# jaredhuling/oem

Measured on NVIDIA B200. Metric: full lambda-path fit time, lower is better.
Workload: dtype f64

## Files before the change

oem_b200/build.py:

```python
import os
import subprocess
import sys

HERE = os.path.dirname(os.path.abspath(__file__))
CSRC = os.path.join(HERE, "csrc")
LIBDIR = os.path.join(HERE, "lib")
LIB = os.path.join(LIBDIR, "liboem_b200.so")
SOURCES = ["runtime.cu", "gram_syrk.cu", "colstats.cu", "assemble.cu", "path_kernel.cu", "host_common.cu",
           "entries.cu", "entry_logistic.cu", "entry_xval.cu", "entry_xval_logistic.cu", "entry_sparse.cu", "cvscore.cu", "logit_slab.cu", "comm.cu", "ingest.cu"]
NVCC_FLAGS = ["-gencode", "arch=compute_100a,code=sm_100a", "-lineinfo", "-O3", "-std=c++17",
              "-Xcompiler", "-fPIC", "-Xcompiler", "-O2"]


def _stale(target, deps):
    if not os.path.exists(target):
        return True
    t = os.path.getmtime(target)
    return any(os.path.getmtime(d) > t for d in deps)


def build(force=False, verbose=False):
    nvcc = os.environ.get("NVCC", "/usr/local/cuda/bin/nvcc")
    os.makedirs(LIBDIR, exist_ok=True)
    objdir = os.path.join(HERE, "build")
    os.makedirs(objdir, exist_ok=True)
    headers = [os.path.join(CSRC, f) for f in os.listdir(CSRC) if f.endswith((".h", ".cuh"))]
    headers.append(os.path.join(HERE, "..", "include", "oem_b200.h"))
    srcs = [s for s in SOURCES if os.path.exists(os.path.join(CSRC, s))]
    objs, procs = [], []
    for s in srcs:
        src = os.path.join(CSRC, s)
        obj = os.path.join(objdir, s.replace(".cu", ".o"))
        objs.append(obj)
        if force or _stale(obj, [src] + headers):
            cmd = [nvcc] + NVCC_FLAGS + (["-Xptxas", "-v"] if verbose else []) + ["-c", src, "-o", obj]
            procs.append((s, subprocess.Popen(cmd, stdout=subprocess.PIPE, stderr=subprocess.STDOUT, text=True)))
    failed = False
    for s, pr in procs:
        out, _ = pr.communicate()
        if pr.returncode != 0 or verbose:
            sys.stderr.write(f"--- nvcc {s} ---\n{out}\n")
        failed = failed or pr.returncode != 0
    if failed:
        raise RuntimeError("nvcc failed")
    if procs or force or _stale(LIB, objs):
        cmd = [nvcc, "-shared", "-o", LIB] + objs + ["-gencode", "arch=compute_100a,code=sm_100a"]
        subprocess.check_call(cmd)
    return LIB


if __name__ == "__main__":
    print(build(force="--force" in sys.argv, verbose="-v" in sys.argv))
```

oem_b200/csrc/entries.cu:

```cuda
#include <algorithm>
#include <cmath>
#include <cstdlib>
#include <cstring>
#include "host_common.h"

namespace oemb200 {

thread_local std::string g_last_error;

void check_common(const oemb200_spec *s, const oemb200_opts *o, const oemb200_result *r, const char *want_family,
                  bool allow_weights) {
    if (!s || !o || !r) fail(OEMB200_EINVAL, "spec / opts / result must not be NULL");
    if (!s->family || strcmp(s->family, want_family) != 0) {
        if (strcmp(want_family, "gaussian") == 0)
            fail(OEMB200_EINVAL, "binomial not available for oem_fit_dense, use oem_fit_logistic_dense");
        fail(OEMB200_EINVAL, "family must be \"%s\"", want_family);
    }
    if (s->n_weights > 0 && !allow_weights) fail(OEMB200_EUNSUPPORTED, "weights not implemented yet.");
    if (s->n_weights > 0 && !s->weights) fail(OEMB200_EINVAL, "n_weights > 0 but weights is NULL");
    if (!r->beta || !r->lambda || !r->niter || !r->d) fail(OEMB200_EINVAL, "result buffers beta/lambda/niter/d are required");
    if (o->maxit < 1) fail(OEMB200_EINVAL, "maxit must be >= 1");
}

void to_device_matrix(Ctx &cx, const double *x, int64_t n, int p, int64_t ldx, DevMatrix &m) {
    if (is_device_ptr(x)) { m.p = x; m.ld = ldx; return; }
    size_t free_b = 0, total_b = 0;
    OEM_CUDA(cudaMemGetInfo(&free_b, &total_b));
    m.ld = n + (n & 1);
    const size_t need = (size_t)m.ld * p * 8;
    if (need + (2ull << 30) > free_b)
        fail(OEMB200_EUNSUPPORTED, "x (%.1f GB) does not fit next to the workspace on the device (%.1f GB free); "
             "use oem_fit_big (streams row chunks) or shard the rows over more GPUs", need / 1e9, free_b / 1e9);
    m.own.alloc((size_t)m.ld * p);
    if (m.ld != n) m.own.zero(cx.stream);
    h2d_block(cx, x, ldx, n, p, m.own.p, m.ld, cx.stream);
    m.p = m.own.p;
}
void to_device_vector(Ctx &cx, const double *v, int64_t n, DevVector &d) {
    if (is_device_ptr(v)) { d.p = v; return; }
    d.own.alloc(n + (n & 1));
    d.own.zero(cx.stream);
    d.own.upload(v, n, cx.stream);
    cx.st.h2d_bytes += n * 8;
    d.p = d.own.p;
}

void fill_common_outputs(const Setup &su, oemb200_result *res) {
    const int L = su.Lmax;
    for (int pp = 0; pp < su.P; ++pp) {
        for (int i = 0; i < L; ++i) {
            res->lambda[(size_t)pp * L + i] = i < (int)su.lam[pp].size() ? su.lam[pp][i] : 0.0;
            if (res->loss) res->loss[(size_t)pp * L + i] = 1e99;
        }
        if (res->nlam_out) res->nlam_out[pp] = su.nlam_run[pp];
    }
}

void finish_stats(Ctx &cx, PhaseTimers &tm, size_t total_id, oemb200_result *res) {
    tm.stop(total_id);
    cx.finish();
    if (res->stats) *res->stats = cx.st;
}

static void fit_big(const double *x, int64_t n, int p, int64_t ldx, const double *y, const oemb200_spec *s,
                    const oemb200_opts *o, oemb200_result *res) {
    check_common(s, o, res, "gaussian");
    if (n < 1 || p < 1 || ldx < n) fail(OEMB200_EINVAL, "bad dimensions n=%lld p=%d ldx=%lld", (long long)n, p, (long long)ldx);
    const int icpt = s->intercept ? 1 : 0, q = p + icpt;
    Ctx cx(o);
    PhaseTimers &tm = *cx.tm;
    const size_t t_total = tm.start(&cx.st.ms_total);
    Setup su;
    su.parse(s, q, p, false);

    const size_t nb = (size_t)p * p + 3 * (size_t)p + 3;
    DBuf<double> bundle(nb);
    bundle.zero(cx.stream);
    double *G = bundle.p, *stats = G + (size_t)p * p, *ysum = stats + 3 * (size_t)p, *nobs = ysum + 2;

    DevVector yv;
    to_device_vector(cx, y, n, yv);
    const size_t t_y = tm.start(&cx.st.ms_colstats);
    vecsum_launch(cx, yv.p, n, 0.0, ysum, false);
    tm.stop(t_y);

    const bool fused_stats = getenv("OEMB200_SEPARATE_COLSTATS") == nullptr;
    if (is_device_ptr(x)) {
        if (fused_stats) {
            gram_launch(cx, x, n, p, ldx, {RowSegment{0, n, 0}}, 1, nullptr, nullptr, G, false, yv.p, stats);
        } else {
            const size_t t1 = tm.start(&cx.st.ms_colstats);
            colstats_launch(cx, x, n, p, ldx, nullptr, yv.p, nullptr, stats, false);
            tm.stop(t1);
            gram_launch(cx, x, n, p, ldx, {RowSegment{0, n, 0}}, 1, nullptr, nullptr, G, false);
        }
    } else {
        const double gigs = o->gigs > 0 ? o->gigs : 1.0;
        int64_t rows = (int64_t)(gigs * 1e9 / (8.0 * p));
        const int64_t align = 2 * gram_kt();
        rows = std::max<int64_t>(align, rows / align * align);
        rows = std::min<int64_t>(rows, (n + align - 1) / align * align);
        DBuf<double> stage[2];
        stage[0].alloc((size_t)rows * p);
        stage[1].alloc((size_t)rows * p);
        struct CopyLane {
            cudaStream_t s = nullptr;
            cudaEvent_t ready[2] = {nullptr, nullptr}, freed[2] = {nullptr, nullptr};
            CopyLane() {
                OEM_CUDA(cudaStreamCreateWithFlags(&s, cudaStreamNonBlocking));
                for (int b = 0; b < 2; ++b) {
                    OEM_CUDA(cudaEventCreateWithFlags(&ready[b], cudaEventDisableTiming));
                    OEM_CUDA(cudaEventCreateWithFlags(&freed[b], cudaEventDisableTiming));
                }
            }
            ~CopyLane() {
                if (s) cudaStreamSynchronize(s);
                for (int b = 0; b < 2; ++b) { if (ready[b]) cudaEventDestroy(ready[b]); if (freed[b]) cudaEventDestroy(freed[b]); }
                if (s) cudaStreamDestroy(s);
            }
        } lane;
        cudaStream_t cs = lane.s;
        cudaEvent_t *ready = lane.ready, *freed = lane.freed;
        const int64_t nchunks = (n + rows - 1) / rows;
        const bool pinned_src = is_pinned_host(x);
        auto issue_copy = [&](int64_t c) {
            const int b = (int)(c & 1);
            const int64_t r0 = c * rows, nr = std::min(rows, n - r0);
            if (c >= 2) OEM_CUDA(cudaStreamWaitEvent(cs, freed[b], 0));
            h2d_block(cx, x + r0, ldx, nr, p, stage[b].p, rows, cs);
            OEM_CUDA(cudaEventRecord(ready[b], cs));
        };
        const size_t t_h = tm.start(&cx.st.ms_h2d);
        issue_copy(0);
        if (nchunks > 1 && pinned_src) issue_copy(1);
        for (int64_t c = 0; c < nchunks; ++c) {
            const int b = (int)(c & 1);
            const int64_t r0 = c * rows, nr = std::min(rows, n - r0);
            OEM_CUDA(cudaStreamWaitEvent(cx.stream, ready[b], 0));
            if (fused_stats) {
                gram_launch(cx, stage[b].p, nr, p, rows, {RowSegment{0, nr, 0}}, 1, nullptr, nullptr, G, c > 0, yv.p + r0, stats);
            } else {
                colstats_launch(cx, stage[b].p, nr, p, rows, nullptr, yv.p + r0, nullptr, stats, c > 0);
                gram_launch(cx, stage[b].p, nr, p, rows, {RowSegment{0, nr, 0}}, 1, nullptr, nullptr, G, c > 0);
            }
            OEM_CUDA(cudaEventRecord(freed[b], cx.stream));
            const int64_t nxt = pinned_src ? c + 2 : c + 1;
            if (nxt < nchunks) issue_copy(nxt);
        }
        tm.stop(t_h);
        cx.sync();
    }
    const double nd = (double)n;
    OEM_CUDA(cudaMemcpyAsync(nobs, &nd, 8, cudaMemcpyHostToDevice, cx.stream));
    const size_t t_ar = tm.start(&cx.st.ms_allreduce);
    cx.all_reduce(bundle.p, (int64_t)nb);
    tm.stop(t_ar);

    double n_tot = 0.0;
    OEM_CUDA(cudaMemcpyAsync(&n_tot, nobs, 8, cudaMemcpyDeviceToHost, cx.stream));
    cx.sync();
    if (!(n_tot > q)) fail(OEMB200_EUNSUPPORTED, "n <= p branch (XX' form, src/oem_big.h:363-366) is outside the hot path");

    const size_t t_as = tm.start(&cx.st.ms_assemble);
    DBuf<double> XX((size_t)q * q), XY(q), cinv(p);
    assemble_aug_launch(cx, p, icpt, s->standardize ? 1 : 0, 1, 1, G, stats, ysum, 1, nobs, nobs, XX.p, XY.p, cinv.p, nullptr);
    std::vector<double> hXY(q), hcinv(p);
    XY.download(hXY.data(), q, cx.stream);
    cinv.download(hcinv.data(), p, cx.stream);
    tm.stop(t_as);
    cx.sync();

    double lmax = 0.0;
    for (int j = 0; j < q; ++j) lmax = std::max(lmax, std::fabs(hXY[j]));
    su.build_lambdas(s, lmax, false);

    PenaltyTables tb(cx, su, s, p, icpt);
    PathBuffers pb;
// ... 553 lines not shown
        cudaGetLastError();
        delete m;
    });
}

int oemb200_matrix_info(const oemb200_matrix *m, int64_t *n, int *p, int64_t *ld, const double **dev_ptr, int64_t *h2d_bytes,
                        double *ms_upload) {
    return guarded([&] {
        check_handle(m);
        if (n) *n = m->n;
        if (p) *p = m->p;
        if (ld) *ld = m->ld;
        if (dev_ptr) *dev_ptr = m->dev;
        if (h2d_bytes) *h2d_bytes = m->h2d_bytes;
        if (ms_upload) *ms_upload = m->ms_upload;
    });
}

int oemb200_fit_dense_h(const oemb200_matrix *x, const double *y, const oemb200_spec *spec, const oemb200_opts *opts,
                        oemb200_result *res) {
    return guarded([&] { check_handle(x); HandleOpts h(x, opts); fit_dense(x->dev, x->n, x->p, x->ld, y, spec, &h.o, res); });
}
int oemb200_fit_big_h(const oemb200_matrix *x, const double *y, const oemb200_spec *spec, const oemb200_opts *opts,
                      oemb200_result *res) {
    return guarded([&] { check_handle(x); HandleOpts h(x, opts); fit_big(x->dev, x->n, x->p, x->ld, y, spec, &h.o, res); });
}
int oemb200_fit_logistic_dense_h(const oemb200_matrix *x, const double *y, const oemb200_spec *spec, const oemb200_opts *opts,
                                 oemb200_result *res) {
    return guarded([&] {
        check_handle(x);
        HandleOpts h(x, opts);
        fit_logistic(x->dev, x->n, x->p, x->ld, y, spec, &h.o, res, &x->slab);
    });
}
int oemb200_xval_dense_h(const oemb200_matrix *x, const double *y, const oemb200_spec *spec, int nfolds, const int *foldid,
                         const char *type_measure, const oemb200_opts *opts, oemb200_result *res) {
    return guarded([&] {
        check_handle(x);
        HandleOpts h(x, opts);
        fit_xval(x->dev, x->n, x->p, x->ld, y, spec, nfolds, foldid, type_measure, &h.o, res);
    });
}
int oemb200_xval_logistic_dense_h(const oemb200_matrix *x, const double *y, const oemb200_spec *spec, int nfolds,
                                  const int *foldid, const char *type_measure, const oemb200_opts *opts, oemb200_result *res) {
    return guarded([&] {
        check_handle(x);
        HandleOpts h(x, opts);
        fit_xval_logistic(x->dev, x->n, x->p, x->ld, y, spec, nfolds, foldid, type_measure, &h.o, res);
    });
}
int oemb200_predict_h(const oemb200_matrix *x, const double *beta, int beta_rows, int nlambda, int type, double *out,
                      int64_t ldo, const oemb200_opts *opts, oemb200_stats *stats) {
    return guarded([&] {
        check_handle(x);
        HandleOpts h(x, opts);
        predict_entry(x->dev, x->n, x->p, x->ld, beta, beta_rows, nlambda, type, out, ldo, &h.o, stats);
    });
}

static void phase_ctx_opts(oemb200_opts &o, void *stream) {
    oemb200_default_opts(&o);
    o.stream = stream;
}
static double elapsed_ms(cudaEvent_t a, cudaEvent_t b) {
    float ms = 0.f;
    cudaEventElapsedTime(&ms, a, b);
    return ms;
}
#define OEM_PHASE_TIMED(body)                                                    \
    oemb200_opts o_; phase_ctx_opts(o_, stream);                                 \
    Ctx cx(&o_);                                                                 \
    cudaEvent_t ea, eb;                                                          \
    OEM_CUDA(cudaEventCreate(&ea)); OEM_CUDA(cudaEventCreate(&eb));              \
    OEM_CUDA(cudaEventRecord(ea, cx.stream));                                    \
    body;                                                                        \
    OEM_CUDA(cudaEventRecord(eb, cx.stream));                                    \
    cx.sync();                                                                   \
    if (ms_out) *ms_out = elapsed_ms(ea, eb);                                    \
    cudaEventDestroy(ea); cudaEventDestroy(eb);

int oemb200_gram(const double *x_dev, int64_t n, int p, int64_t ldx, const double *mean_dev, const double *row_w_dev,
                 double *g_dev, void *stream, double *ms_out) {
    return guarded([&] {
        OEM_PHASE_TIMED(gram_launch(cx, x_dev, n, p, ldx, {RowSegment{0, n, 0}}, 1, mean_dev, row_w_dev, g_dev, false));
    });
}
int oemb200_colstats(const double *x_dev, int64_t n, int p, int64_t ldx, const double *v0_dev, const double *v1_dev,
                     double *out_dev, void *stream, double *ms_out) {
    return guarded([&] { OEM_PHASE_TIMED(colstats_launch(cx, x_dev, n, p, ldx, v0_dev, v1_dev, nullptr, out_dev, false)); });
}
int oemb200_xb_logistic(const double *x_dev, int64_t n, int p, int64_t ldx, const double *b_dev, double b0,
                        const double *y_dev, double *prob_dev, double *resid_dev, double *w_dev, void *stream,
                        double *ms_out) {
    return guarded([&] {
        OEM_PHASE_TIMED(xb_launch(cx, x_dev, n, p, ldx, b_dev, b0, y_dev, nullptr, prob_dev, resid_dev, w_dev, true));
    });
}
int oemb200_logit_slab_pass(const double *x_dev, int64_t n, int p, int64_t ldx, const double *b_dev, double b0,
                            const double *y_dev, double *prob_dev, double *w_dev, double *grad_dev, int reps, void *stream,
                            double *ms_out, double *ms_relayout_out) {
    return guarded([&] {
        if (!x_dev || !b_dev || !y_dev || !grad_dev || n < 1 || p < 1 || ldx < n) fail(OEMB200_EINVAL, "logit_slab_pass: bad arguments");
        if (!logit_slab_rows(p)) fail(OEMB200_EUNSUPPORTED, "the slab kernel covers 8 <= p <= 2048 (p = %d)", p);
        oemb200_opts o_; phase_ctx_opts(o_, stream);
        Ctx cx(&o_);
        cudaEvent_t e0, e1, e2;
        OEM_CUDA(cudaEventCreate(&e0)); OEM_CUDA(cudaEventCreate(&e1)); OEM_CUDA(cudaEventCreate(&e2));
        DBuf<double> slabs(logit_slab_doubles(n, p)), d_b0(1);
        OEM_CUDA(cudaMemcpyAsync(d_b0.p, &b0, 8, cudaMemcpyHostToDevice, cx.stream));
        OEM_CUDA(cudaEventRecord(e0, cx.stream));
        logit_slab_relayout(cx, x_dev, n, p, ldx, slabs.p);
        OEM_CUDA(cudaEventRecord(e1, cx.stream));
        const int nrep = reps < 1 ? 1 : reps;
        for (int r = 0; r < nrep; ++r) logit_slab_launch(cx, slabs.p, n, p, b_dev, d_b0.p, y_dev, prob_dev, w_dev, grad_dev);
        OEM_CUDA(cudaEventRecord(e2, cx.stream));
        cx.sync();
        if (ms_relayout_out) *ms_relayout_out = elapsed_ms(e0, e1);
        if (ms_out) *ms_out = elapsed_ms(e1, e2) / nrep;
        cudaEventDestroy(e0); cudaEventDestroy(e1); cudaEventDestroy(e2);
    });
}
int oemb200_logit_fold_pass(const double *x_dev, int64_t n, int p, int64_t ldx, const double *b_dev, const double *b0_dev,
                            const double *y_dev, const int *fold_dev, int M, const int *conv_dev, double *grad_dev, int reps,
                            void *stream, double *ms_out, double *ms_relayout_out, int *sweeps_out) {
    return guarded([&] {
        if (!x_dev || !b_dev || !b0_dev || !y_dev || !fold_dev || !grad_dev || n < 1 || p < 1 || ldx < n || M < 1)
            fail(OEMB200_EINVAL, "logit_fold_pass: bad arguments");
        if (!logit_fold_models(p)) fail(OEMB200_EUNSUPPORTED, "the fused fold pass covers 8 <= p <= 2048 (p = %d)", p);
        oemb200_opts o_; phase_ctx_opts(o_, stream);
        Ctx cx(&o_);
        cudaEvent_t e0, e1, e2;
        OEM_CUDA(cudaEventCreate(&e0)); OEM_CUDA(cudaEventCreate(&e1)); OEM_CUDA(cudaEventCreate(&e2));
        DBuf<double> slabs(logit_fold_doubles(n, p));
        OEM_CUDA(cudaEventRecord(e0, cx.stream));
        logit_fold_relayout(cx, x_dev, n, p, ldx, slabs.p);
        OEM_CUDA(cudaEventRecord(e1, cx.stream));
        const int nrep = reps < 1 ? 1 : reps;
        int sweeps = 0;
        for (int r = 0; r < nrep; ++r)
            sweeps = logit_fold_launch(cx, slabs.p, n, p, b_dev, b0_dev, y_dev, fold_dev, M, conv_dev, nullptr, nullptr, grad_dev);
        OEM_CUDA(cudaEventRecord(e2, cx.stream));
        cx.sync();
        if (ms_relayout_out) *ms_relayout_out = elapsed_ms(e0, e1);
        if (ms_out) *ms_out = elapsed_ms(e1, e2) / nrep;
        if (sweeps_out) *sweeps_out = sweeps;
        cudaEventDestroy(e0); cudaEventDestroy(e1); cudaEventDestroy(e2);
    });
}
int oemb200_top_eig(const double *xx_dev, int q, double *lambda_max_out, int *steps_out, void *stream) {
    return guarded([&] {
        oemb200_opts o_; phase_ctx_opts(o_, stream);
        Ctx cx(&o_);
        DBuf<double> d(1), xy(q);
        DBuf<int> lz(1);
        xy.zero(cx.stream);
        PathProblem pp;
        pp.q = q; pp.ngram = 1; pp.XX = xx_dev; pp.XY = xy.p; pp.d = d.p; pp.compute_eig = true;
        pp.eig_factor = 1.0; pp.eig_tol = 1e-10; pp.Lmax = 1; pp.lanczos_steps = lz.p;
        path_launch(cx, pp);
        double h; int k;
        d.download(&h, 1, cx.stream);
        lz.download(&k, 1, cx.stream);
        cx.sync();
        if (lambda_max_out) *lambda_max_out = h;
        if (steps_out) *steps_out = k;
    });
}
// ... 3 lines not shown
```

oem_b200/csrc/gram_syrk.cu:

```cuda
#include <algorithm>
#include <functional>
#include <cstdlib>
#include <type_traits>
#include <mutex>
#include "runtime.h"

namespace oemb200 {

constexpr int G_TILE = 128;
constexpr int G_KT = 36;
constexpr int G_KSTEPS = G_KT / 4;
constexpr int G_STAGES = 3;
constexpr int G_CWARPS = 8;
constexpr int G_THREADS = G_CWARPS * 32;
constexpr int G_PANEL = G_TILE * G_KT;
constexpr int G_PANEL_BYTES = G_PANEL * 8;
constexpr int G_STAGE_BYTES = 2 * G_PANEL_BYTES;
constexpr int G_SMEM_BYTES = G_STAGES * G_STAGE_BYTES + 128;

int gram_kt() { return G_KT; }

struct GramItem {
    int pi, pj, slot, pad;
    long long row0, row1;
// ... 277 lines not shown
                    so[e * G_TILE + rlo * 8 + g] = st_lo[e];
                    so[e * G_TILE + rhi * 8 + g] = st_hi[e];
                }
            }
        }
        double *slot = ws + (size_t)it.slot * (G_TILE * G_TILE);
#pragma unroll
        for (int sl = 0; sl < 17; ++sl) {
            const int row = sl <= warp ? rlo : rhi;
            const int col = sl <= warp ? sl : sl - warp - 1;
            const int i = row * 8 + g, j = col * 8 + 2 * t;
            slot[(size_t)j * G_TILE + i] = acc[sl][0];
            slot[(size_t)(j + 1) * G_TILE + i] = acc[sl][1];
        }
    }
}

__global__ void __launch_bounds__(256)
gram_reduce_kernel(const double *__restrict__ ws, const GramTile *__restrict__ tiles, double *__restrict__ G, int q,
                   int accumulate) {
    const GramTile tl = tiles[blockIdx.y];
    const int e = blockIdx.x * 256 + threadIdx.x;
    const int i = e & (G_TILE - 1), j = e >> 7;
    const int gi = tl.pi * G_TILE + i, gj = tl.pj * G_TILE + j;
    if (gi >= q || gj >= q || gi < gj) return;
    const double *p = ws + (size_t)tl.slot0 * (G_TILE * G_TILE) + e;
    double s = 0.0;
    for (int k = 0; k < tl.nslots; ++k) s += p[(size_t)k * (G_TILE * G_TILE)];
    double *Go = G + (size_t)tl.out * q * q;
    if (accumulate) s += Go[(size_t)gj * q + gi];
    Go[(size_t)gj * q + gi] = s;
    Go[(size_t)gi * q + gj] = s;
}

__global__ void gram_stats_reduce_kernel(const double *__restrict__ stats_ws, const int *__restrict__ chunk_out, int nchunks,
                                         int npanels, int q, int nout, const double *__restrict__ G,
                                         double *__restrict__ stats_out, int accumulate) {
    const int j = blockIdx.x * blockDim.x + threadIdx.x;
    const int o = blockIdx.y;
    if (j >= q) return;
    const int pi = j / G_TILE, jl = j - pi * G_TILE;
    double s[2] = {0.0, 0.0};
    for (int c = 0; c < nchunks; ++c) {
        if (chunk_out[c] != o) continue;
        const double *so = stats_ws + ((size_t)c * npanels + pi) * (2 * G_TILE) + jl;
#pragma unroll
        for (int e = 0; e < 2; ++e) s[e] += so[e * G_TILE];
    }
    double *out = stats_out + (size_t)o * 3 * q;
#pragma unroll
    for (int e = 0; e < 2; ++e) out[(size_t)e * q + j] = accumulate ? out[(size_t)e * q + j] + s[e] : s[e];
    out[(size_t)2 * q + j] = G[(size_t)o * q * q + (size_t)j * q + j];
}

typedef CUresult (*EncodeTiledFn)(CUtensorMap *, CUtensorMapDataType, cuuint32_t, void *, const cuuint64_t *,
                                  const cuuint64_t *, const cuuint32_t *, const cuuint32_t *, CUtensorMapInterleave,
                                  CUtensorMapSwizzle, CUtensorMapL2promotion, CUtensorMapFloatOOBfill);

static EncodeTiledFn get_encode_fn() {
    static EncodeTiledFn fn = nullptr;
    static std::once_flag once;
    std::call_once(once, [] {
        void *p = nullptr;
        cudaDriverEntryPointQueryResult qres;
        if (cudaGetDriverEntryPoint("cuTensorMapEncodeTiled", &p, cudaEnableDefault, &qres) == cudaSuccess &&
            qres == cudaDriverEntryPointSuccess)
            fn = reinterpret_cast<EncodeTiledFn>(p);
    });
    return fn;
}

template <bool C, bool W, bool T, bool S>
static void launch_variant(Ctx &cx, const CUtensorMap &tm, const double *X, int64_t ld, int64_t n, int q,
                           const GramItem *d_items, int nitems, const double *mean, const double *roww, double *ws,
                           const double *yvec, double *stats_ws, int npanels) {
    auto kern = gram_syrk_kernel<C, W, T, S>;
    OEM_CUDA(cudaFuncSetAttribute(kern, cudaFuncAttributeMaxDynamicSharedMemorySize, G_SMEM_BYTES));
    kern<<<nitems, G_THREADS, G_SMEM_BYTES, cx.stream>>>(tm, X, ld, n, q, d_items, mean, roww, ws, yvec, stats_ws, npanels);
    OEM_CUDA(cudaGetLastError());
}

void gram_launch(Ctx &cx, const double *X, int64_t n, int q, int64_t ld, const std::vector<RowSegment> &segs,
                 int nout, const double *mean, const double *roww, double *G, bool accumulate, const double *stats_y,
                 double *stats_out) {
    if (stats_out && roww) fail(OEMB200_EINVAL, "gram: fused column statistics are not available with row weights");
    if (n <= 0 || q <= 0) fail(OEMB200_EINVAL, "gram: empty matrix (n=%lld, p=%d)", (long long)n, q);
    if (n >= (1ll << 31)) fail(OEMB200_EINVAL, "gram: more than 2^31-1 rows per call; shard or chunk the rows");
    const int P = (q + G_TILE - 1) / G_TILE;
    const int ntile_pairs = P * (P + 1) / 2;

    int64_t rows_total = 0;
    for (auto &s : segs) {
        if (s.row0 < 0 || s.row1 > n || s.row1 < s.row0 || s.out < 0 || s.out >= nout)
            fail(OEMB200_EINVAL, "gram: bad row segment");
        if ((s.row0 % G_KT) != 0 && s.row0 != 0) fail(OEMB200_EINVAL, "gram: segment start not a multiple of %d", G_KT);
        if (((s.row1 - s.row0) % G_KT) != 0 && s.row1 != n)
            fail(OEMB200_EINVAL, "gram: interior segment length not a multiple of %d", G_KT);
        rows_total += s.row1 - s.row0;
    }
    const int64_t min_rows = 32 * G_KT;
    auto round_chunk = [&](int64_t target_chunks) {
        int64_t cr = (rows_total + target_chunks - 1) / std::max<int64_t>(1, target_chunks);
        return std::max<int64_t>(min_rows, ((cr + G_KT - 1) / G_KT) * G_KT);
    };
    int64_t chunk_rows;
    if (const char *e = getenv("OEMB200_GRAM_WAVES")) {
        chunk_rows = round_chunk(std::max<int64_t>(1, (int64_t)std::max(1, atoi(e)) * cx.num_sms / ntile_pairs));
    } else {
        const bool partial = (q % G_TILE) != 0;
        const int nfull = partial ? (P - 1) * (P - 2) / 2 : P * (P - 1) / 2;
        const int nlast = partial ? P - 1 : 0;
        const double cost_last = partial ? (8.0 + std::max(0, std::min(8, (q - (P - 1) * G_TILE - 64 + 7) / 8)) +
                                            std::min(8, (q - (P - 1) * G_TILE + 7) / 8) - 8.0) / 16.0 : 1.0;
        const double cost_diag = stats_out ? 0.60 : 0.54;
        auto makespan = [&](int64_t cr) {
            std::vector<double> cost;
            std::vector<double> len;
            for (auto &sg : segs) {
                const int64_t l = sg.row1 - sg.row0;
                if (l <= 0) continue;
                const int64_t nc = (l + cr - 1) / cr;
                const int64_t per = (((l + nc - 1) / nc) + G_KT - 1) / G_KT * G_KT;
                for (int64_t r = 0; r < l; r += per) len.push_back((double)((std::min(l, r + per) - r + G_KT - 1) / G_KT) + 3.0);
            }
            for (double c : {1.0, cost_last, cost_diag}) {
                const int nt = c == 1.0 ? nfull : (c == cost_diag ? P : nlast);
                for (double l : len)
                    for (int t = 0; t < nt; ++t) cost.push_back(l * c);
            }
            std::vector<double> sm(cx.num_sms, 0.0);
            std::make_heap(sm.begin(), sm.end(), std::greater<double>());
            double end = 0.0;
            for (double c : cost) {
                std::pop_heap(sm.begin(), sm.end(), std::greater<double>());
                sm.back() += c;
                end = std::max(end, sm.back());
                std::push_heap(sm.begin(), sm.end(), std::greater<double>());
            }
            return end;
        };
        const int64_t c_lo = std::max<int64_t>(1, (int64_t)6 * cx.num_sms / ntile_pairs);
        const int64_t c_hi = std::max<int64_t>(c_lo, (int64_t)14 * cx.num_sms / ntile_pairs);
        chunk_rows = round_chunk(c_lo);
        double best = makespan(chunk_rows);
        for (int64_t c = c_lo + 1; c <= c_hi; ++c) {
            const int64_t cr = round_chunk(c);
            if (cr == chunk_rows) continue;
            const double m = makespan(cr);
            if (m < best * 0.999) { best = m; chunk_rows = cr; }
        }
    }
    const int64_t max_slots = (1536ll << 20) / (G_TILE * G_TILE * 8);
    for (;;) {
        int64_t nchunks = 0;
        for (auto &s : segs) nchunks += std::max<int64_t>(1, (s.row1 - s.row0 + chunk_rows - 1) / chunk_rows);
        if (nchunks * ntile_pairs <= max_slots) break;
        chunk_rows *= 2;
    }

    std::vector<GramItem> items;
    std::vector<GramTile> tiles;
    std::vector<int> chunks_per_out(nout, 0);
    struct Chunk { int64_t r0, r1; int out, idx; };
    std::vector<Chunk> chunks;
    for (auto &s : segs) {
        const int64_t len = s.row1 - s.row0;
        if (len == 0) continue;
        const int64_t nc = (len + chunk_rows - 1) / chunk_rows;
        int64_t per = (((len + nc - 1) / nc) + G_KT - 1) / G_KT * G_KT;
        for (int64_t r = s.row0; r < s.row1; r += per) {
// ... 105 lines not shown
```

oem_b200/csrc/runtime.h:

```cpp
#pragma once
#include <cuda_runtime.h>
#include <cstdint>
#include <cstring>
#include <string>
#include <array>
#include <vector>
#include "../../include/oem_b200.h"
#include "common.cuh"

namespace oemb200 {

cudaEvent_t event_acquire();
void event_release(cudaEvent_t e);

struct PhaseTimers {
    struct Rec { cudaEvent_t a, b; double *acc; };
    std::vector<Rec> recs;
    cudaStream_t s;
    bool off = getenv("OEMB200_NO_PHASE_TIMERS") != nullptr;
    explicit PhaseTimers(cudaStream_t s_) : s(s_) {}
    PhaseTimers(const PhaseTimers &) = delete;
    ~PhaseTimers() { for (auto &r : recs) { event_release(r.a); event_release(r.b); } }
    size_t start(double *acc) {
        if (off) return 0;
// ... 28 lines not shown

    explicit Ctx(const oemb200_opts *o);
    ~Ctx();
    void sync() { st.host_syncs += 1; OEM_CUDA(cudaStreamSynchronize(stream)); }
    bool distributed() const { return comm != nullptr || allreduce != nullptr; }
    void all_reduce(double *dev_buf, int64_t count, const int *skip = nullptr, unsigned long long *t_acc = nullptr);
    bool all_reduce_can_skip(int64_t count) const;
    void finish();
};

void *pool_alloc(size_t bytes);
void pool_free(void *p);
void pool_release_all();

template <typename T>
struct DBuf {
    T *p = nullptr;
    size_t n = 0;
    DBuf() {}
    explicit DBuf(size_t n_) { alloc(n_); }
    DBuf(const DBuf &) = delete;
    DBuf &operator=(const DBuf &) = delete;
    DBuf(DBuf &&o) noexcept : p(o.p), n(o.n) { o.p = nullptr; o.n = 0; }
    DBuf &operator=(DBuf &&o) noexcept {
        if (this != &o) { release(); p = o.p; n = o.n; o.p = nullptr; o.n = 0; }
        return *this;
    }
    ~DBuf() { release(); }
    void alloc(size_t n_) {
        release();
        n = n_;
        if (n) p = static_cast<T *>(pool_alloc(n * sizeof(T)));
    }
    void release() {
        if (p) pool_free(p);
        p = nullptr;
        n = 0;
    }
    void zero(cudaStream_t s) { if (n) OEM_CUDA(cudaMemsetAsync(p, 0, n * sizeof(T), s)); }
    void upload(const T *h, size_t cnt, cudaStream_t s) {
        OEM_CUDA(cudaMemcpyAsync(p, h, cnt * sizeof(T), cudaMemcpyHostToDevice, s));
    }
    void download(T *h, size_t cnt, cudaStream_t s) const {
        OEM_CUDA(cudaMemcpyAsync(h, p, cnt * sizeof(T), cudaMemcpyDeviceToHost, s));
    }
};

bool is_device_ptr(const void *p);

template <typename F>
void collective_guard(Ctx &cx, F &&f) {
    int code = 0;
    std::string msg;
    try {
        f();
    } catch (const Error &e) {
        code = e.code;
        msg = e.what();
    }
    if (cx.distributed()) {
        DBuf<double> flag(1);
        double h = code ? 1.0 : 0.0;
        flag.upload(&h, 1, cx.stream);
        cx.sync();
        cx.all_reduce(flag.p, 1);
        flag.download(&h, 1, cx.stream);
        cx.sync();
        if (h > 0.0 && !code) fail(OEMB200_ECOMM, "another rank rejected its inputs; this rank stops before the next collective");
    }
    if (code) throw Error(code, msg);
}

bool is_pinned_host(const void *p);
void h2d_block(Ctx &cx, const double *src, int64_t ldx, int64_t nr, int p, double *dst, int64_t ld_dst, cudaStream_t stream);
void release_host_stager();

void comm_all_reduce(oemb200_comm *c, double *dev_buf, int64_t count, cudaStream_t stream, const int *skip = nullptr,
                     unsigned long long *t_acc = nullptr);
bool comm_can_skip(const oemb200_comm *c, int64_t count);

struct RowSegment { int64_t row0, row1; int out; };
void gram_launch(Ctx &cx, const double *X, int64_t n, int q, int64_t ld, const std::vector<RowSegment> &segs,
                 int nout, const double *mean, const double *roww, double *G, bool accumulate,
                 const double *stats_y = nullptr, double *stats_out = nullptr);
int gram_kt();

void colstats_launch(Ctx &cx, const double *X, int64_t n, int p, int64_t ld, const double *v0, const double *v1,
                     const double *shift, double *out3p, bool accumulate);
void vecsum_launch(Ctx &cx, const double *v, int64_t n, double shift, double *out2, bool accumulate);
void affine_launch(Ctx &cx, const double *v, int64_t n, double shift, double divisor, double *out);
void axpy_launch(Ctx &cx, int64_t n, double a, const double *x, double *y);
void xb_launch(Ctx &cx, const double *X, int64_t n, int p, int64_t ld, const double *b, double b0, const double *y,
               double *eta, double *prob, double *resid, double *w, bool logistic, const double *b0_dev = nullptr);

struct ChainDesc {
    int gram;
    int penalty;
    int nlam;
    int lam_off;
    double alpha, gamma, tau;
    int out_off;
};
struct PathScratch;
PathScratch *path_scratch_create();
void path_scratch_destroy(PathScratch *s);

struct PathProblem {
    int q = 0;
    int ngram = 0;
    const double *XX = nullptr;
    const double *XY = nullptr;
    double *d = nullptr;
    bool compute_eig = true;
    double eig_factor = 1.005;
    double eig_tol = 1e-11;
    std::vector<ChainDesc> chains;
    const double *lambdas = nullptr;
    int Lmax = 0;
    const double *pen_fact = nullptr;
    int ngroups = 0;
    int ngidx = 0;
    const int *unique_groups = nullptr, *grp_ptr = nullptr, *grp_idx = nullptr;
    const double *group_weights = nullptr;
    const int *grp_cover = nullptr;
    const double *post_scale = nullptr;
    const double *beta_init = nullptr;
    double *beta_final = nullptr;
    int maxit = 500;
    double tol = 1e-7;
    bool accelerate = false;
    double *beta_out = nullptr;
    int *niter_out = nullptr;
    int *lanczos_steps = nullptr;
    PathScratch *scratch = nullptr;
    const int *skip = nullptr;
    int *irls_conv = nullptr;
    volatile int *irls_host_flag = nullptr;
    long long *irls_iters_total = nullptr;
    double irls_tol = 0.0;
    const double *irls_cinv = nullptr;
    int irls_p = 0, irls_icpt = 0;
    double *irls_b = nullptr, *irls_b0 = nullptr;
    unsigned long long *t_acc = nullptr;
    const double *xy_grad = nullptr, *xy_cinv = nullptr;
    double xy_n = 0.0;
    int xy_icpt = 0;
    double *xy_out = nullptr;
};
void path_launch(Ctx &cx, const PathProblem &pp);
void path_xy_launch(Ctx &cx, int q, int icpt, const double *XX, const double *beta, const double *g, const double *cinv, double n_tot,
                    double *XY, const int *skip);
void path_check_fits(Ctx &cx, int q, int chains_per_gram, int Lmax, int ngroups, int ngidx);

void assemble_aug_launch(Ctx &cx, int p, int intercept, int standardize, int nparts, int nout,
                         const double *G_parts , const double *stats_parts ,
                         const double *ysum_parts , int ysum_stride,
                         const double *corner_parts ,
                         const double *nobs_parts , double *XX , double *XY ,
                         double *colsq_inv , double *nobs_out );
void assemble_dense_launch(Ctx &cx, int p, int flag, double n, const double *G, const double *xy, const double *css,
                           double *XX, double *XY, double *scalex);
void scale_sym_launch(Ctx &cx, int p, const double *sinv, const double *XXin, const double *XYin, double *XX,
                      double *XY);
void symv_add_launch(Ctx &cx, int q, const double *M, const double *x, const double *add, double *y);

int logit_slab_rows(int p);
bool logit_slab_preferred(int64_t n, int p);
size_t logit_slab_doubles(int64_t n, int p);
// ... 30 lines not shown
```

Baseline: 0.3664.

## Add int8 split-plane tcgen05 Gram path emulating f64 for large inputs

```diff
diff --git a/oem_b200/build.py b/oem_b200/build.py
--- a/oem_b200/build.py
+++ b/oem_b200/build.py
@@ -6,7 +6,7 @@
 CSRC = os.path.join(HERE, "csrc")
 LIBDIR = os.path.join(HERE, "lib")
 LIB = os.path.join(LIBDIR, "liboem_b200.so")
-SOURCES = ["runtime.cu", "gram_syrk.cu", "colstats.cu", "assemble.cu", "path_kernel.cu", "host_common.cu",
+SOURCES = ["runtime.cu", "gram_syrk.cu", "gram_i8.cu", "colstats.cu", "assemble.cu", "path_kernel.cu", "host_common.cu",
            "entries.cu", "entry_logistic.cu", "entry_xval.cu", "entry_xval_logistic.cu", "entry_sparse.cu", "cvscore.cu", "logit_slab.cu", "comm.cu", "ingest.cu"]
 NVCC_FLAGS = ["-gencode", "arch=compute_100a,code=sm_100a", "-lineinfo", "-O3", "-std=c++17",
               "-Xcompiler", "-fPIC", "-Xcompiler", "-O2"]
diff --git a/oem_b200/csrc/entries.cu b/oem_b200/csrc/entries.cu
--- a/oem_b200/csrc/entries.cu
+++ b/oem_b200/csrc/entries.cu
@@ -87,12 +87,12 @@
     const bool fused_stats = getenv("OEMB200_SEPARATE_COLSTATS") == nullptr;
     if (is_device_ptr(x)) {
         if (fused_stats) {
-            gram_launch(cx, x, n, p, ldx, {RowSegment{0, n, 0}}, 1, nullptr, nullptr, G, false, yv.p, stats);
+            gram_launch(cx, x, n, p, ldx, {RowSegment{0, n, 0}}, 1, nullptr, nullptr, G, false, yv.p, stats, true);
         } else {
             const size_t t1 = tm.start(&cx.st.ms_colstats);
             colstats_launch(cx, x, n, p, ldx, nullptr, yv.p, nullptr, stats, false);
             tm.stop(t1);
-            gram_launch(cx, x, n, p, ldx, {RowSegment{0, n, 0}}, 1, nullptr, nullptr, G, false);
+            gram_launch(cx, x, n, p, ldx, {RowSegment{0, n, 0}}, 1, nullptr, nullptr, G, false, nullptr, nullptr, true);
         }
     } else {
         const double gigs = o->gigs > 0 ? o->gigs : 1.0;
@@ -812,7 +812,8 @@
 int oemb200_gram(const double *x_dev, int64_t n, int p, int64_t ldx, const double *mean_dev, const double *row_w_dev,
                  double *g_dev, void *stream, double *ms_out) {
     return guarded([&] {
-        OEM_PHASE_TIMED(gram_launch(cx, x_dev, n, p, ldx, {RowSegment{0, n, 0}}, 1, mean_dev, row_w_dev, g_dev, false));
+        OEM_PHASE_TIMED(gram_launch(cx, x_dev, n, p, ldx, {RowSegment{0, n, 0}}, 1, mean_dev, row_w_dev, g_dev, false, nullptr,
+                                    nullptr, true));
     });
 }
 int oemb200_colstats(const double *x_dev, int64_t n, int p, int64_t ldx, const double *v0_dev, const double *v1_dev,
diff --git a/oem_b200/csrc/gram_i8.cu b/oem_b200/csrc/gram_i8.cu
--- /dev/null
+++ b/oem_b200/csrc/gram_i8.cu
@@ -0,0 +1,361 @@
+#include <cstdlib>
+#include <cstring>
+#include "runtime.h"
+
+namespace oemb200 {
+
+constexpr int I8_S = 8;
+constexpr int I8_TM = 128;
+constexpr int I8_TN = 64;
+constexpr int I8_KT = 32;
+constexpr int I8_STAGES = 4;
+constexpr int I8_A_BYTES = I8_TM * I8_KT;
+constexpr int I8_B_BYTES = I8_TN * I8_KT;
+constexpr int I8_STAGE_BYTES = I8_S * (I8_A_BYTES + I8_B_BYTES);
+constexpr int I8_SMEM_BYTES = I8_STAGES * I8_STAGE_BYTES + 1024 + 256;
+constexpr int I8_DRAIN_STAGES = 1024;
+constexpr int I8_EPI_WARPS = 8;
+constexpr int I8_THREADS = (I8_EPI_WARPS + 2) * 32;
+constexpr int64_t I8_CHUNK = 1 << 20;
+constexpr int I8_TMEM_COLS = (I8_S) * I8_TN;
+static_assert(I8_TMEM_COLS <= 512, "levels 2 .. S + 1 must fit the 512 TMEM columns");
+
+constexpr int I8_PRE_THREADS = 256;
+
+__global__ void __launch_bounds__(I8_PRE_THREADS)
+i8_prepass_kernel(const double *__restrict__ X, long long ld, long long n, int p, long long rows_per_block,
+                  const double *__restrict__ y, double *__restrict__ part) {
+    const int j = blockIdx.x;
+    const long long r0 = (long long)blockIdx.y * rows_per_block;
+    const long long r1 = min(n, r0 + rows_per_block);
+    const double *col = X + (size_t)j * ld;
+    double mx = 0.0, sx = 0.0, sxy = 0.0;
+    for (long long r = r0 + threadIdx.x; r < r1; r += I8_PRE_THREADS) {
+        const double x = __ldcs(col + r);
+        mx = fmax(mx, fabs(x));
+        sx += x;
+        if (y) sxy = fma(x, __ldg(y + r), sxy);
+    }
+    __shared__ double sh[3][I8_PRE_THREADS / 32];
+    for (int o = 16; o > 0; o >>= 1) {
+        mx = fmax(mx, __shfl_xor_sync(0xffffffffu, mx, o));
+        sx += __shfl_xor_sync(0xffffffffu, sx, o);
+        sxy += __shfl_xor_sync(0xffffffffu, sxy, o);
+    }
+    const int w = threadIdx.x >> 5;
+    if ((threadIdx.x & 31) == 0) { sh[0][w] = mx; sh[1][w] = sx; sh[2][w] = sxy; }
+    __syncthreads();
+    if (threadIdx.x == 0) {
+        for (int k = 1; k < I8_PRE_THREADS / 32; ++k) { mx = fmax(mx, sh[0][k]); sx += sh[1][k]; sxy += sh[2][k]; }
+        double *o = part + ((size_t)blockIdx.y * p + j) * 3;
+        o[0] = mx; o[1] = sx; o[2] = sxy;
+    }
+}
+
+__global__ void i8_prepass_finish_kernel(const double *__restrict__ part, int nblk, int p, int *__restrict__ exps,
+                                         double *__restrict__ stats_out) {
+    const int j = blockIdx.x * blockDim.x + threadIdx.x;
+    if (j >= p) return;
+    double mx = 0.0, sx = 0.0, sxy = 0.0;
+    for (int b = 0; b < nblk; ++b) {
+        const double *o = part + ((size_t)b * p + j) * 3;
+        mx = fmax(mx, o[0]); sx += o[1]; sxy += o[2];
+    }
+    int e = 0;
+    if (mx > 0.0) frexp(mx, &e);
+    exps[j] = e;
+    if (stats_out) { stats_out[j] = sx; stats_out[(size_t)p + j] = sxy; }
+}
+
+constexpr int I8_SPLIT_ROWS = 1024;
+
+__global__ void __launch_bounds__(256)
+i8_split_kernel(const double *__restrict__ X, long long ld, long long r0, long long nr, int p,
+                const int *__restrict__ exps, int8_t *__restrict__ planes, long long Rpad, int Ppad) {
+    const int c = blockIdx.y;
+    const double scale = c < p ? ldexp(1.0, 6 - exps[c]) : 0.0;
+    const double *col = X + (size_t)min(c, p - 1) * ld + r0;
+    const int sw = (c >> 2) & 1;
+#pragma unroll
+    for (int k = 0; k < I8_SPLIT_ROWS / 256; ++k) {
+        const long long r = (long long)blockIdx.x * I8_SPLIT_ROWS + k * 256 + threadIdx.x;
+        if (r >= Rpad) break;
+        double v = (c < p && r < nr) ? __ldcs(col + r) * scale : 0.0;
+        const int rr = (int)(r & (I8_KT - 1));
+        int8_t *dst = planes + ((size_t)(r >> 5) * I8_S * Ppad + c) * I8_KT + ((((rr >> 4) ^ sw)) << 4) + (rr & 15);
+#pragma unroll
+        for (int a = 0; a < I8_S; ++a) {
+            const double d = rint(v);
+            dst[(size_t)a * Ppad * I8_KT] = static_cast<int8_t>(static_cast<int>(d));
+            v = (v - d) * 128.0;
+        }
+    }
+}
+
+__device__ __forceinline__ uint64_t i8_sdesc(uint32_t saddr) {
+    uint64_t d = (uint64_t)((saddr & 0x3FFFFu) >> 4);
+    d |= (uint64_t)1 << 16;
+    d |= (uint64_t)(256 >> 4) << 32;
+    d |= (uint64_t)1 << 46;
+    d |= (uint64_t)6 << 61;
+    return d;
+}
+__host__ __device__ constexpr uint32_t i8_idesc(int N) {
+    return (2u << 4)
+         | (1u << 7) | (1u << 10)
+         | ((uint32_t)(N >> 3) << 17)
+         | ((uint32_t)(I8_TM >> 4) << 24);
+}
+__device__ __forceinline__ void i8_mma(uint32_t d_tmem, uint64_t a, uint64_t b, uint32_t idesc) {
+    asm volatile("{\n\t.reg .pred p;\n\tsetp.ne.b32 p, 1, 0;\n\t"
+                 "tcgen05.mma.cta_group::1.kind::i8 [%0], %1, %2, %3, p;\n\t}"
+                 ::"r"(d_tmem), "l"(a), "l"(b), "r"(idesc) : "memory");
+}
+__device__ __forceinline__ void i8_commit(uint64_t *bar) {
+    asm volatile("tcgen05.commit.cta_group::1.mbarrier::arrive::one.shared::cluster.b64 [%0];"
+                 ::"r"(smem_u32(bar)) : "memory");
+}
+__device__ __forceinline__ void bulk_load(void *dst, const void *src, uint32_t bytes, uint64_t *bar) {
+    asm volatile("cp.async.bulk.shared::cluster.global.mbarrier::complete_tx::bytes [%0], [%1], %2, [%3];"
+                 ::"r"(smem_u32(dst)), "l"(src), "r"(bytes), "r"(smem_u32(bar)) : "memory");
+}
+__device__ __forceinline__ void tc_fence_before() { asm volatile("tcgen05.fence::before_thread_sync;" ::: "memory"); }
+__device__ __forceinline__ void tc_fence_after() { asm volatile("tcgen05.fence::after_thread_sync;" ::: "memory"); }
+
+__device__ __forceinline__ void tmem_ld16(uint32_t taddr, uint32_t (&v)[16]) {
+    asm volatile("tcgen05.ld.sync.aligned.32x32b.x16.b32 {%0,%1,%2,%3,%4,%5,%6,%7,%8,%9,%10,%11,%12,%13,%14,%15}, [%16];"
+                 : "=r"(v[0]), "=r"(v[1]), "=r"(v[2]), "=r"(v[3]), "=r"(v[4]), "=r"(v[5]), "=r"(v[6]), "=r"(v[7]),
+                   "=r"(v[8]), "=r"(v[9]), "=r"(v[10]), "=r"(v[11]), "=r"(v[12]), "=r"(v[13]), "=r"(v[14]), "=r"(v[15])
+                 : "r"(taddr));
+    asm volatile("tcgen05.wait::ld.sync.aligned;" ::: "memory");
+}
+__device__ __forceinline__ void tmem_zero16(uint32_t taddr) {
+    const uint32_t z = 0;
+    asm volatile("tcgen05.st.sync.aligned.32x32b.x16.b32 [%0], {%1,%1,%1,%1,%1,%1,%1,%1,%1,%1,%1,%1,%1,%1,%1,%1};"
+                 ::"r"(taddr), "r"(z) : "memory");
+}
+
+__global__ void __launch_bounds__(I8_THREADS, 1)
+i8_syrk_kernel(const int8_t *__restrict__ planes, int Ppad, int ntiles, long long range_rows, long long nrows,
+               double *__restrict__ ws, int accumulate) {
+    extern __shared__ unsigned char smem_raw[];
+    const uint32_t raw = smem_u32(smem_raw);
+    unsigned char *smem = smem_raw + (((raw + 1023u) & ~1023u) - raw);
+    uint64_t *full = reinterpret_cast<uint64_t *>(smem + I8_STAGES * I8_STAGE_BYTES);
+    uint64_t *empty = full + I8_STAGES;
+    uint64_t *tmem_full = empty + I8_STAGES;
+    uint64_t *tmem_empty = tmem_full + 1;
+    uint32_t *tmem_slot = reinterpret_cast<uint32_t *>(tmem_empty + 1);
+
+    const int warp = threadIdx.x >> 5, lane = threadIdx.x & 31;
+    const int tile = blockIdx.x % ntiles, range = blockIdx.x / ntiles;
+    int pi = 0;
+    while ((pi + 1) * (pi + 2) <= tile) ++pi;
+    const int pj = tile - pi * (pi + 1);
+    const long long row0 = (long long)range * range_rows;
+    const long long row1 = min(nrows, row0 + range_rows);
+    const int nk = row1 > row0 ? (int)((row1 - row0 + I8_KT - 1) / I8_KT) : 0;
+    const int ndrain = (nk + I8_DRAIN_STAGES - 1) / I8_DRAIN_STAGES;
+
+    if (threadIdx.x == 0) {
+        for (int s = 0; s < I8_STAGES; ++s) { mbar_init(&full[s], 1); mbar_init(&empty[s], 1); }
+        mbar_init(tmem_full, 1);
+        mbar_init(tmem_empty, I8_EPI_WARPS);
+        mbar_fence_init();
+    }
+    if (warp == 0) {
+        asm volatile("tcgen05.alloc.cta_group::1.sync.aligned.shared::cta.b32 [%0], %1;"
+                     ::"r"(smem_u32(tmem_slot)), "r"(I8_TMEM_COLS) : "memory");
+        asm volatile("tcgen05.relinquish_alloc_permit.cta_group::1.sync.aligned;" ::: "memory");
+    }
+    tc_fence_before();
+    __syncthreads();
+    tc_fence_after();
+    const uint32_t tmem = *tmem_slot;
+
+    if (warp == I8_EPI_WARPS) {
+        if (lane == 0) {
+            for (int kt = 0; kt < nk; ++kt) {
+                const int s = kt % I8_STAGES;
+                if (kt >= I8_STAGES) mbar_wait(&empty[s], ((kt / I8_STAGES) - 1) & 1);
+                unsigned char *st = smem + (size_t)s * I8_STAGE_BYTES;
+                mbar_arrive_expect_tx(&full[s], I8_STAGE_BYTES);
+                const int8_t *blk = planes + (size_t)((row0 >> 5) + kt) * I8_S * Ppad * I8_KT;
+#pragma unroll
+                for (int a = 0; a < I8_S; ++a) {
+                    const int8_t *pl = blk + (size_t)a * Ppad * I8_KT;
+                    bulk_load(st + a * I8_A_BYTES, pl + pi * I8_A_BYTES, I8_A_BYTES, &full[s]);
+                    bulk_load(st + I8_S * I8_A_BYTES + a * I8_B_BYTES, pl + pj * I8_B_BYTES, I8_B_BYTES, &full[s]);
+                }
+            }
+        }
+    } else if (warp == I8_EPI_WARPS + 1) {
+        if (lane == 0) {
+            int drain = 0;
+            for (int kt = 0; kt < nk; ++kt) {
+                const int s = kt % I8_STAGES;
+                if (kt % I8_DRAIN_STAGES == 0) {
+                    mbar_wait(tmem_empty, drain & 1);
+                    tc_fence_after();
+                }
+                mbar_wait(&full[s], (kt / I8_STAGES) & 1);
+                tc_fence_after();
+                const uint32_t sa = smem_u32(smem + (size_t)s * I8_STAGE_BYTES);
+                const uint32_t sb = sa + I8_S * I8_A_BYTES;
+#pragma unroll
+                for (int a = 1; a <= I8_S; ++a) {
+                    const uint64_t da = i8_sdesc(sa + (a - 1) * I8_A_BYTES);
+#pragma unroll
+                    for (int b = 1, w = 4; b <= I8_S + 1 - a; b += w) {
+                        while (b + w - 1 > I8_S + 1 - a) w >>= 1;
+                        i8_mma(tmem + (uint32_t)(I8_TN * (a + b - 2)), da, i8_sdesc(sb + (b - 1) * I8_B_BYTES),
+                               i8_idesc(I8_TN * w));
+                    }
+                }
+                i8_commit(&empty[s]);
+                if (kt % I8_DRAIN_STAGES == I8_DRAIN_STAGES - 1 || kt == nk - 1) {
+                    i8_commit(tmem_full);
+                    ++drain;
+                }
+            }
+        }
+    } else {
+        constexpr int JW = I8_TN / 2;
+        const int quarter = warp & 3, j0w = (warp >> 2) * JW;
+        const uint32_t tl = tmem + ((uint32_t)(quarter * 32) << 16) + (uint32_t)j0w;
+        auto zero_tmem = [&] {
+#pragma unroll
+            for (int L = 2; L <= I8_S + 1; ++L)
+#pragma unroll
+                for (int c = 0; c < JW; c += 16) tmem_zero16(tl + (uint32_t)(I8_TN * (L - 2) + c));
+            asm volatile("tcgen05.wait::st.sync.aligned;" ::: "memory");
+            tc_fence_before();
+            __syncwarp();
+            if (lane == 0) mbar_arrive(tmem_empty);
+        };
+        double acc[JW];
+#pragma unroll
+        for (int j = 0; j < JW; ++j) acc[j] = 0.0;
+        if (nk > 0) zero_tmem();
+        for (int d = 0; d < ndrain; ++d) {
+            mbar_wait(tmem_full, d & 1);
+            tc_fence_after();
+#pragma unroll
+            for (int c0 = 0; c0 < JW; c0 += 16) {
+                double t[16];
+#pragma unroll
+                for (int k = 0; k < 16; ++k) t[k] = 0.0;
+#pragma unroll 1
+                for (int L = I8_S + 1; L >= 2; --L) {
+                    uint32_t v[16];
+                    tmem_ld16(tl + (uint32_t)(I8_TN * (L - 2) + c0), v);
+#pragma unroll
+                    for (int k = 0; k < 16; ++k) t[k] = fma(t[k], 0x1p-7, (double)(int)v[k]);
+                }
+#pragma unroll
+                for (int k = 0; k < 16; ++k) acc[c0 + k] += t[k];
+            }
+            if (d + 1 < ndrain) zero_tmem();
+        }
+        double *slot = ws + (size_t)blockIdx.x * (I8_TM * I8_TN) + (size_t)j0w * I8_TM + quarter * 32 + lane;
+#pragma unroll
+        for (int j = 0; j < JW; ++j) {
+            double v = acc[j];
+            if (accumulate) v += slot[(size_t)j * I8_TM];
+            slot[(size_t)j * I8_TM] = v;
+        }
+    }
+    tc_fence_before();
+    __syncthreads();
+    if (warp == 0) {
+        tc_fence_after();
+        asm volatile("tcgen05.dealloc.cta_group::1.sync.aligned.b32 %0, %1;" ::"r"(tmem), "r"(I8_TMEM_COLS) : "memory");
+    }
+}
+
+__global__ void __launch_bounds__(256)
+i8_reduce_kernel(const double *__restrict__ ws, int ntiles, int nranges, const int *__restrict__ exps, int q,
+                 double *__restrict__ G, double *__restrict__ stats_out) {
+    const int tile = blockIdx.y;
+    int pi = 0;
+    while ((pi + 1) * (pi + 2) <= tile) ++pi;
+    const int pj = tile - pi * (pi + 1);
+    const int e = blockIdx.x * 256 + threadIdx.x;
+    const int i = e & (I8_TM - 1), j = e >> 7;
+    const int gi = pi * I8_TM + i, gj = pj * I8_TN + j;
+    if (gi >= q || gj >= q || gi < gj) return;
+    double s = 0.0;
+    for (int r = 0; r < nranges; ++r) s += ws[((size_t)r * ntiles + tile) * (I8_TM * I8_TN) + e];
+    s = ldexp(s, exps[gi] + exps[gj] - 12);
+    G[(size_t)gj * q + gi] = s;
+    G[(size_t)gi * q + gj] = s;
+    if (stats_out && gi == gj) stats_out[(size_t)2 * q + gi] = s;
+}
+
+int gram_i8_route() {
+    const char *e = getenv("OEMB200_GRAM_ROUTE");
+    if (!e || !*e) return -1;
+    if (!strcmp(e, "dmma")) return 0;
+    if (!strcmp(e, "i8")) return 1;
+    fail(OEMB200_EINVAL, "OEMB200_GRAM_ROUTE must be 'dmma' or 'i8' (got '%s')", e);
+}
+
+bool gram_i8_default(int64_t n, int q) {
+    if (n < (1ll << 20) || q < 768) return false;
+    const size_t Ppad = (size_t)(q + I8_TM - 1) / I8_TM * I8_TM;
+    const size_t need = (size_t)I8_S * Ppad * (size_t)std::min<int64_t>(I8_CHUNK, n) + (512ull << 20);
+    size_t free_b = 0, total_b = 0;
+    return cudaMemGetInfo(&free_b, &total_b) == cudaSuccess && need <= free_b;
+}
+
+void gram_i8_launch(Ctx &cx, const double *X, int64_t n, int q, int64_t ld, double *G, const double *stats_y,
+                    double *stats_out) {
+    const int P = (q + I8_TM - 1) / I8_TM;
+    const int Ppad = P * I8_TM;
+    const int ntiles = P * (P + 1);
+    const int64_t chunk = std::min<int64_t>(I8_CHUNK, n);
+    const int64_t nchunks = (n + chunk - 1) / chunk;
+    const int64_t rpad_max = (chunk + 63) / 64 * 64;
+    int nranges = std::max(1, cx.num_sms / ntiles);
+    nranges = (int)std::min<int64_t>(nranges, std::max<int64_t>(1, rpad_max / 4096));
+    const int64_t range_rows = ((rpad_max + nranges - 1) / nranges + I8_KT - 1) / I8_KT * I8_KT;
+    nranges = (int)((rpad_max + range_rows - 1) / range_rows);
+
+    const int64_t rows_per_block = std::max<int64_t>(65536, (n + 63) / 64);
+    const int nblk = (int)((n + rows_per_block - 1) / rows_per_block);
+    DBuf<double> part((size_t)nblk * q * 3);
+    DBuf<int> exps(q);
+    DBuf<int8_t> planes((size_t)I8_S * Ppad * rpad_max);
+    DBuf<double> ws((size_t)nranges * ntiles * I8_TM * I8_TN);
+    const size_t t_pre = cx.tm->start(&cx.st.ms_colstats);
+    i8_prepass_kernel<<<dim3(q, nblk), I8_PRE_THREADS, 0, cx.stream>>>(X, ld, n, q, rows_per_block, stats_y, part.p);
+    OEM_CUDA(cudaGetLastError());
+    i8_prepass_finish_kernel<<<(q + 127) / 128, 128, 0, cx.stream>>>(part.p, nblk, q, exps.p, stats_out);
+    OEM_CUDA(cudaGetLastError());
+    cx.tm->stop(t_pre);
+
+    OEM_CUDA(cudaFuncSetAttribute(i8_syrk_kernel, cudaFuncAttributeMaxDynamicSharedMemorySize, I8_SMEM_BYTES));
+
+    for (int64_t c = 0; c < nchunks; ++c) {
+        const int64_t r0 = c * chunk, nr = std::min(chunk, n - r0);
+        const size_t t_s = cx.tm->start(&cx.st.ms_colstats);
+        dim3 sg((unsigned)((rpad_max + I8_SPLIT_ROWS - 1) / I8_SPLIT_ROWS), (unsigned)Ppad);
+        i8_split_kernel<<<sg, 256, 0, cx.stream>>>(X, ld, r0, nr, q, exps.p, planes.p, rpad_max, Ppad);
+        OEM_CUDA(cudaGetLastError());
+        cx.tm->stop(t_s);
+        const size_t t_k = cx.tm->start(&cx.st.ms_gram);
+        i8_syrk_kernel<<<nranges * ntiles, I8_THREADS, I8_SMEM_BYTES, cx.stream>>>(planes.p, Ppad, ntiles, range_rows, nr, ws.p,
+                                                                                  c > 0 ? 1 : 0);
+        OEM_CUDA(cudaGetLastError());
+        cx.tm->stop(t_k);
+    }
+    const size_t t_r = cx.tm->start(&cx.st.ms_gram_reduce);
+    i8_reduce_kernel<<<dim3(I8_TM * I8_TN / 256, ntiles), 256, 0, cx.stream>>>(ws.p, ntiles, nranges, exps.p, q, G, stats_out);
+    OEM_CUDA(cudaGetLastError());
+    cx.tm->stop(t_r);
+    cx.st.kernel_launches += 3 + 2 * nchunks;
+    cx.st.gram_launches += 1;
+    cx.st.gram_flops += (double)n * q * (q + 1.0);
+}
+
+}
diff --git a/oem_b200/csrc/gram_syrk.cu b/oem_b200/csrc/gram_syrk.cu
--- a/oem_b200/csrc/gram_syrk.cu
+++ b/oem_b200/csrc/gram_syrk.cu
@@ -383,10 +383,15 @@
 
 void gram_launch(Ctx &cx, const double *X, int64_t n, int q, int64_t ld, const std::vector<RowSegment> &segs,
                  int nout, const double *mean, const double *roww, double *G, bool accumulate, const double *stats_y,
-                 double *stats_out) {
+                 double *stats_out, bool allow_i8) {
     if (stats_out && roww) fail(OEMB200_EINVAL, "gram: fused column statistics are not available with row weights");
     if (n <= 0 || q <= 0) fail(OEMB200_EINVAL, "gram: empty matrix (n=%lld, p=%d)", (long long)n, q);
     if (n >= (1ll << 31)) fail(OEMB200_EINVAL, "gram: more than 2^31-1 rows per call; shard or chunk the rows");
+    if (allow_i8 && !mean && !roww && !accumulate && nout == 1 && segs.size() == 1 && segs[0].row0 == 0 &&
+        segs[0].row1 == n && gram_i8_route() != 0 && (gram_i8_route() == 1 || gram_i8_default(n, q))) {
+        gram_i8_launch(cx, X, n, q, ld, G, stats_y, stats_out);
+        return;
+    }
     const int P = (q + G_TILE - 1) / G_TILE;
     const int ntile_pairs = P * (P + 1) / 2;
 
diff --git a/oem_b200/csrc/runtime.h b/oem_b200/csrc/runtime.h
--- a/oem_b200/csrc/runtime.h
+++ b/oem_b200/csrc/runtime.h
@@ -134,8 +134,13 @@
 struct RowSegment { int64_t row0, row1; int out; };
 void gram_launch(Ctx &cx, const double *X, int64_t n, int q, int64_t ld, const std::vector<RowSegment> &segs,
                  int nout, const double *mean, const double *roww, double *G, bool accumulate,
-                 const double *stats_y = nullptr, double *stats_out = nullptr);
+                 const double *stats_y = nullptr, double *stats_out = nullptr, bool allow_i8 = false);
 int gram_kt();
+
+int gram_i8_route();
+bool gram_i8_default(int64_t n, int q);
+void gram_i8_launch(Ctx &cx, const double *X, int64_t n, int q, int64_t ld, double *G, const double *stats_y,
+                    double *stats_out);
 
 void colstats_launch(Ctx &cx, const double *X, int64_t n, int p, int64_t ld, const double *v0, const double *v1,
                      const double *shift, double *out3p, bool accumulate);
```

Result: faster. 0.3151 (median of 6 runs) (-14.0%).
